# google/neural-light-transport

Hardware: AMD Instinct MI355X
Metric: rendered Mtexels/s at 1024^2 UV (full Model.call forward: U-Net + UV->camera warp); at N > 1: N collective-free replicas of this forward (weak scaling).  The data-parallel TRAIN step with the RCCL gradient all-reduce (BASELINE config 4) is `train_step`: value = Mtexels/s over all ranks, speedup_vs_o (higher is better)
Workload: dtype f32 via 3xbf16 split, 9 exact products, fp32 accumulate (the LDS-tiled encoder convs: fp32 operands as three bf16 terms on v_mfma_f32_16x16x32_bf16, every term product exact in fp32); f32 storage everywhere, every other launch native f32; 1 GPU; BASELINE config 3: dragon_specular relight+view-synth, depth0 16/depth 256, 4 frames/GPU, 1024^2 UV, k=4 obs maps, 512^2 camera warp; frames_per_gpu=4, uv=1024, k=4, cam=512, conv_algo=auto, plan=fused ends, launch=eager, two HIP streams, distinct_batches_rotated=3, launch_tape_replays=0, parallelism=dp1 (frames sharded, no forward collective), world=1, dist_world_size=1, device=cuda:0

## Files before the change

neural-light-transport_amd/_capi.py:

```python
import ctypes
import threading
import os

import torch

_HERE = os.path.dirname(os.path.abspath(__file__))
LIB_PATH = os.environ.get('NLT_HIP_LIB') or os.path.join(_HERE, 'libnlt_hip.so')

CONV1X1, CONV_K2S2, CONV_K2S1, DECONV_K2S2, DECONV_K2S1 = range(5)
CONV_K3S1, CONV_K3S2, DECONV_K3S1, DECONV_K3S2 = range(5, 9)
ALGO_AUTO, ALGO_DIRECT, ALGO_MFMA = range(3)

_c_int, _c_long, _c_float, _vp = ctypes.c_int, ctypes.c_long, ctypes.c_float, ctypes.c_void_p
_c_double = ctypes.c_double
MAP_F64, MAP_F32, MAP_F16 = range(3)

SIGNATURES = {
    'nlt_version': (ctypes.c_char_p, []),
    'nlt_status_string': (ctypes.c_char_p, [_c_int]),
    'nlt_packed_weight_floats': (_c_long, [_c_int] * 4),
    'nlt_pack_conv_weights': (_c_int, [_c_int, _vp, _c_int, _c_int, _c_int, _vp, _vp]),
    'nlt_conv_forward': (_c_int, [_c_int, _c_int, _c_int, _vp, _c_int, _c_int, _vp, _c_int, _c_int,
                                  _c_int, _c_int, _c_int, _vp, _vp, _vp, _c_int, _vp, _c_int,
                                  _c_int, _c_float, _vp, _c_int, _c_int, _vp]),
# ... 828 lines not shown


NORM_LAYER, NORM_BATCH = 0, 1


def norm_forward(kind, x, gamma, beta, mean, var, eps):
    c = x.shape[-1]
    y = torch.empty_like(x)
    _call('nlt_norm_forward', kind, _ptr(_dense(x, 'x')), x.numel() // c, c, _ptr(gamma), _ptr(beta), _ptr(mean), _ptr(var),
          float(eps), _ptr(y))
    return y


def norm_backward(kind, g, x, gamma, mean, var, eps, dgamma, dbeta):
    _same_shape(g, x, 'norm_backward')
    c = x.shape[-1]
    texels = x.numel() // c
    ws = _workspace('norm', x.device, _size('nlt_norm_workspace_floats', texels, c, what='the kernel takes c <= 1024'))
    dx = torch.empty_like(x)
    _call('nlt_norm_backward', kind, _ptr(_dense(g, 'g')), _ptr(_dense(x, 'x')), texels, c, _ptr(gamma), _ptr(mean), _ptr(var),
          float(eps), _ptr(dx), _ptr(dgamma), _ptr(dbeta), _ptr(ws))
    return dx


def pool2x2_forward(x, kind):
    n, h, w, c = x.shape
    y = torch.empty((n, h // 2, w // 2, c), device=x.device, dtype=torch.float32)
    _call('nlt_pool2x2_forward', _ptr(_dense(x, 'x')), n, h, w, c, kind, _ptr(y))
    return y


def pool2x2_backward(g, x, kind):
    n, h, w, c = x.shape
    if tuple(g.shape) != (n, h // 2, w // 2, c):
        raise NLTError("pool2x2_backward: gradient %s for input %s" % (tuple(g.shape), tuple(x.shape)))
    dx = torch.empty_like(x)
    _call('nlt_pool2x2_backward', _ptr(_dense(g, 'g')), _ptr(_dense(x, 'x')), n, h, w, c, kind, _ptr(dx))
    return dx


def clip_by_norm_slots(grad, slots, clipnorm):
    _call('nlt_clip_by_norm_slots', _ptr(grad), _tptr(slots, torch.int64, 'slots'), slots.shape[0], float(clipnorm))


def adam_amsgrad_step(param, grad, m, v, vhat, lr_t, beta1, beta2, eps):
    _call('nlt_adam_amsgrad_step', _ptr(param), _ptr(grad), _ptr(m), _ptr(v), _ptr(vhat), param.numel(), float(lr_t), float(beta1),
          float(beta2), float(eps))


def _splitk_workspace(mode, n, h, w, cout, ksplit, device, always=False):
    if abs(ksplit) <= 1 and not always:
        return None
    need = _size('nlt_conv_splitk_workspace_floats', mode, n, h, w, cout, ksplit)
    return _workspace((_stream(), getattr(_tls, 'scope', 0)), device, need, zero=True)


def conv_forward_splitk(mode, ksplit, src0, c0, ld0, src1, c1, ld1, n, h, w, w_packed, bias, cout, out, ldo,
                        act=True, alpha=0.3, tile_hint=0, mask_src=None, ldm=0, accumulate=False):
    ws = _splitk_workspace(mode, n, h, w, cout, ksplit, src0.device, always=True)
    _call('nlt_conv_forward_splitk', mode, tile_hint, ksplit, _ptr(ws), _ptr(src0), ld0, c0, _ptr(src1), ld1, c1, n, h, w,
          _ptr(w_packed), _ptr(bias), cout, _ptr(out), ldo, 1 if act else 0, float(alpha), _ptr(mask_src), ldm,
          1 if accumulate else 0)


def conv_forward_map(mode, ksplit, src0, c0, ld0, src1, c1, ld1, n, h, w, w_packed, bias, cout, out, ldo, bias_map,
                     act=True, alpha=0.3, tile_hint=0, w_keras=None):
    ws = _splitk_workspace(mode, n, h, w, cout, ksplit, src0.device)
    _call('nlt_conv_forward_map', mode, tile_hint, ksplit, _ptr(ws), _ptr(src0), ld0, c0, _ptr(src1), ld1, c1, n, h, w,
          _ptr(w_packed), _ptr(bias), cout, _ptr(out), ldo, 1 if act else 0, float(alpha), _ptr(_dense(bias_map, 'bias_map')),
          bias_map.shape[0])


def conv_backward_data(adj_mode, dpre, cpre, ldp, n, h, w, w_packed, zero_bias, cout, out, ldo, mask_src=None, ldm=0,
                       mask_alpha=0.3, accumulate=False, tile_hint=0, ksplit=1, split=None, w_keras=None):
    ws = _splitk_workspace(adj_mode, n, h, w, cout, ksplit, dpre.device)
    sc, sy, sd, sa, sp = split if split is not None else (0, None, None, 0.0, False)
    _call('nlt_conv_backward_data', adj_mode, tile_hint, ksplit, _ptr(ws), _ptr(dpre), ldp, cpre, n, h, w, _ptr(w_packed),
          _ptr(zero_bias), cout, _ptr(out), ldo, _ptr(mask_src), ldm, float(mask_alpha), 1 if accumulate else 0, sc, _ptr(sy),
          _ptr(sd), float(sa), 1 if sp else 0)


REPACK_MFMA, REPACK_TILE, REPACK_WINO, REPACK_TILE3S2 = 0, 1, 2, 3
REPACK_FIELDS = [('src', 'u8'), ('dst', 'u8'), ('total', 'i8'), ('first_block', 'i8'), ('kind', 'i4'), ('mode', 'i4'),
                 ('c0', 'i4'), ('c1', 'i4'), ('cout', 'i4'), ('tn', 'i4'), ('lo', 'i4'), ('full', 'i4')]


def repack_table(entries, device):
    import numpy as np
    tab = np.zeros(len(entries), dtype=np.dtype(REPACK_FIELDS))
    blocks = 0
    for i, e in enumerate(entries):
        nbytes = e['dst'].numel() * e['dst'].element_size()
        if nbytes % 16 or e['dst'].data_ptr() % 16:
            raise NLTError("repack_table: a packed buffer must be 16-byte aligned and a multiple of 4 floats long")
        tab[i] = (e['src'].data_ptr(), e['dst'].data_ptr(), nbytes // 4, blocks, e['kind'], e['mode'], e['c0'], e['c1'],
                  e['cout'], e['tn'], e['lo'], e['full'])
        blocks += (nbytes // 4 + 255) // 256
    return torch.from_numpy(tab.view(np.uint8)).to(device), len(entries), blocks


def repack_weights(table, n_desc, total_blocks):
    _call('nlt_repack_weights', _tptr(table, torch.uint8, 'repack table'), n_desc, total_blocks)


def conv_tile_supported(mode, cin, cout, tn):
    return lib().nlt_conv_tile_packed_floats(mode, cin, cout, tn) > 0

# ... 393 lines not shown
```

neural-light-transport_amd/csrc/conv_mfma.hip:

```cpp
#include "nlt_common.h"
#include "pack_common.h"

namespace {

typedef __attribute__((address_space(1))) unsigned gu32;

__host__ __device__ inline int chunks16(int c) { return (c + 15) >> 4; }

template <int MODE>
__device__ __forceinline__ int keras_widx(int t, int c, int ncol, int cin, int cout) {
  if (MODE == NLT_CONV1X1 || MODE == NLT_CONV_K2S2 || MODE == NLT_CONV_K2S1) return (t * cin + c) * cout + ncol;
  if (MODE == NLT_DECONV_K2S1) return (t * cout + ncol) * cin + c;
  return ncol * cin + c;
}

template <int MODE>
__global__ void pack_weights_kernel(const float* __restrict__ wk, int c0, int c1, int cout, int N,
                                    int ntiles, long total, float* __restrict__ wp) {
  const long idx = (long)blockIdx.x * blockDim.x + threadIdx.x;
  if (idx >= total) return;
  wp[idx] = nlt_mfma_fragment<MODE>(wk, idx, c0, c1, cout, N, ntiles, cout, 0);
}

template <int MODE>
// ... 106 lines not shown
        for (int rt = 0; rt < RT; ++rt)
#pragma unroll
          for (int ct = 0; ct < CT; ++ct)
            acc[rt][ct] = __builtin_amdgcn_mfma_f32_16x16x4f32(a_cur[ct][s4], b_cur[rt][s4], acc[rt][ct], 0, 0, 0);
#pragma unroll
      for (int ct = 0; ct < CT; ++ct) a_cur[ct] = a_nxt[ct];
#pragma unroll
      for (int rt = 0; rt < RT; ++rt) b_cur[rt] = b_nxt[rt];
    }

  } else {
    f32x4 af[PF][CT], bf[PF][RT];
    int t_n = kbeg / cps, r_n = kbeg - t_n * cps;
    int kload = kbeg;
    if (kbeg < kend) set_tap(t_n);
    auto issue = [&](f32x4 (&a)[CT], f32x4 (&b)[RT]) {
      const bool live = kload < kend;
      if (live && kload > kbeg) {
        if (++r_n == cps) { r_n = 0; set_tap(++t_n); }
      }
      load_frags(r_n, live ? kload : kend - 1, a, b);
      if (!live) {
#pragma unroll
        for (int rt = 0; rt < RT; ++rt) b[rt] = (f32x4){0.f, 0.f, 0.f, 0.f};
      }
      ++kload;
    };
    auto compute = [&](const f32x4 (&a)[CT], const f32x4 (&b)[RT]) {
#pragma unroll
      for (int s4 = 0; s4 < 4; ++s4)
#pragma unroll
        for (int rt = 0; rt < RT; ++rt)
#pragma unroll
          for (int ct = 0; ct < CT; ++ct)
            acc[rt][ct] = __builtin_amdgcn_mfma_f32_16x16x4f32(a[ct][s4], b[rt][s4], acc[rt][ct], 0, 0, 0);
    };
    if (kbeg < kend) {
#pragma unroll
      for (int j = 0; j < PF - 1; ++j) issue(af[j], bf[j]);
      for (int kc = kbeg; kc < kend; kc += PF) {
#pragma unroll
        for (int j = 0; j < PF; ++j) {
          issue(af[(j + PF - 1) % PF], bf[(j + PF - 1) % PF]);
          compute(af[j], bf[j]);
        }
      }
    }

  }
  if constexpr (SPLIT) {
    __shared__ f32x4 red[(NW - 1) * RT * CT * 64 + 1];
    const int kgroups = (ksplit + NW - 1) / NW;
    auto meet = [&]() {
      if (wv) {
#pragma unroll
        for (int rt = 0; rt < RT; ++rt)
#pragma unroll
          for (int ct = 0; ct < CT; ++ct) red[((wv - 1) * RT * CT + rt * CT + ct) * 64 + lane] = acc[rt][ct];
      }
      __syncthreads();
      if (!wv) {
#pragma unroll
        for (int j = 0; j < NW - 1; ++j)
#pragma unroll
          for (int rt = 0; rt < RT; ++rt)
#pragma unroll
            for (int ct = 0; ct < CT; ++ct) acc[rt][ct] += red[(j * RT * CT + rt * CT + ct) * 64 + lane];
      }
    };
    meet();
    if (kgroups > 1) {
      gu32* cnt = (gu32*)ws;
      float* slabs = ws + NLT_SPLITK_COUNTERS;
      const int npad = ntiles * 16;
      const size_t slab = (size_t)p.M * npad;
      if (!wv) {
#pragma unroll
        for (int ct = 0; ct < CT; ++ct) {
          const int ncol = (ng * CT + ct) * 16 + kk * 4;
#pragma unroll
          for (int rt = 0; rt < RT; ++rt)
            if (rv[rt]) *reinterpret_cast<f32x4*>(slabs + (size_t)kg * slab + (size_t)rm[rt] * npad + ncol) = acc[rt][ct];
        }
      }
      asm volatile("s_waitcnt vmcnt(0)" ::: "memory");
      __syncthreads();
      int* flag = reinterpret_cast<int*>(&red[(NW - 1) * RT * CT * 64]);
      if (threadIdx.x == 0) {
        __builtin_amdgcn_fence(__ATOMIC_RELEASE, "agent");
        asm volatile("s_waitcnt vmcnt(0)" ::: "memory");
        const unsigned t = __hip_atomic_fetch_add(cnt + tile, 1u, __ATOMIC_RELAXED, __HIP_MEMORY_SCOPE_AGENT);
        const int last = t == (unsigned)(kgroups - 1);
        if (last) __builtin_amdgcn_fence(__ATOMIC_ACQUIRE, "agent");
        *flag = last;
      }
      __syncthreads();
      if (!*flag) return;
#pragma unroll
      for (int rt = 0; rt < RT; ++rt)
#pragma unroll
        for (int ct = 0; ct < CT; ++ct) acc[rt][ct] = (f32x4){0.f, 0.f, 0.f, 0.f};
#pragma unroll(NW == 4 ? 4 : 1)
      for (int g = wv; g < kgroups; g += NW) {
#pragma unroll
        for (int ct = 0; ct < CT; ++ct) {
          const int ncol = (ng * CT + ct) * 16 + kk * 4;
#pragma unroll
          for (int rt = 0; rt < RT; ++rt)
            acc[rt][ct] += *reinterpret_cast<const f32x4*>(slabs + (size_t)g * slab + (size_t)rm[rt] * npad + ncol);
        }
      }
      meet();
      if (threadIdx.x == 0) __hip_atomic_store(cnt + tile, 0u, __ATOMIC_RELAXED, __HIP_MEMORY_SCOPE_AGENT);
    }
    if (wv) return;
  }

  if constexpr (!SPLIT) {
    if (ksplit > 1) {
      float* part = ws + NLT_SPLITK_COUNTERS;
      const int npad = ntiles * 16;
#pragma unroll
      for (int ct = 0; ct < CT; ++ct) {
        const int ncol = (ng * CT + ct) * 16 + kk * 4;
#pragma unroll
        for (int rt = 0; rt < RT; ++rt)
          if (rv[rt]) *reinterpret_cast<f32x4*>(part + ((size_t)ks * p.M + rm[rt]) * npad + ncol) = acc[rt][ct];
      }
      return;
    }
  }

#pragma unroll
  for (int ct = 0; ct < CT; ++ct) {
    const int ncol = (ng * CT + ct) * 16 + kk * 4;
    if (ncol >= p.N) continue;
    int oc = ncol, ab = 0;
    if (MODE == NLT_DECONV_K2S2) { ab = ncol / p.cout; oc = ncol - ab * p.cout; }
    const f32x4 bv = *reinterpret_cast<const f32x4*>(p.bias + oc);
#pragma unroll
    for (int rt = 0; rt < RT; ++rt) {
      if (!rv[rt]) continue;
      int otex = rm[rt];
      if (MODE == NLT_DECONV_K2S2) otex = (rf[rt] * p.oh + 2 * ry[rt] + (ab >> 1)) * p.ow + 2 * rx[rt] + (ab & 1);
      f32x4 v = acc[rt][ct] + bv;
      if (p.bmap) v += *reinterpret_cast<const f32x4*>(p.bmap + (size_t)(p.bmap_mod ? otex % p.bmap_mod : otex) * p.cout + oc);
      f32x4* o = reinterpret_cast<f32x4*>(p.out + (size_t)otex * p.ldo + oc);
      if (p.accumulate) v += *o;
      if (p.split_c && oc >= p.split_c) { split_store(p, otex, oc, v); continue; }
      if (p.mask_src) {
        const f32x4 mk = *reinterpret_cast<const f32x4*>(p.mask_src + (size_t)otex * p.ldm + oc);
#pragma unroll
        for (int j = 0; j < 4; ++j) v[j] *= (mk[j] > 0.f) ? 1.f : p.alpha;
      } else if (p.act) {
#pragma unroll
        for (int j = 0; j < 4; ++j) v[j] = v[j] > 0.f ? v[j] : p.alpha * v[j];
      }
      *o = v;
    }
  }
}

template <int MODE>
__device__ __forceinline__ void splitk_finish(const ConvP& p, int m, int ncol, f32x4 v) {
  int oc = ncol, ab = 0;
  if (MODE == NLT_DECONV_K2S2) { ab = ncol / p.cout; oc = ncol - ab * p.cout; }
  int otex = m;
  if (MODE == NLT_DECONV_K2S2) {
    const int x = m % p.gw, y = (m / p.gw) % p.gh, f = m / (p.gw * p.gh);
    otex = (f * p.oh + 2 * y + (ab >> 1)) * p.ow + 2 * x + (ab & 1);
  }
  v += *reinterpret_cast<const f32x4*>(p.bias + oc);
  if (p.bmap) v += *reinterpret_cast<const f32x4*>(p.bmap + (size_t)(p.bmap_mod ? otex % p.bmap_mod : otex) * p.cout + oc);
  f32x4* o = reinterpret_cast<f32x4*>(p.out + (size_t)otex * p.ldo + oc);
  if (p.accumulate) v += *o;
  if (p.split_c && oc >= p.split_c) { split_store(p, otex, oc, v); return; }
  if (p.mask_src) {
    const f32x4 mk = *reinterpret_cast<const f32x4*>(p.mask_src + (size_t)otex * p.ldm + oc);
#pragma unroll
    for (int j = 0; j < 4; ++j) v[j] *= (mk[j] > 0.f) ? 1.f : p.alpha;
  } else if (p.act) {
#pragma unroll
    for (int j = 0; j < 4; ++j) v[j] = v[j] > 0.f ? v[j] : p.alpha * v[j];
  }
  *o = v;
}

template <int MODE>
__global__ __launch_bounds__(256) void splitk_epilogue_kernel(ConvP p, int ntiles, int ksplit, const float* __restrict__ ws0) {
  const float* __restrict__ ws = ws0 + NLT_SPLITK_COUNTERS;
  const int quads = p.N >> 2;
  const long idx = (long)blockIdx.x * blockDim.x + threadIdx.x;
  if (idx >= (long)p.M * quads) return;
  const int m = idx / quads;
  const int ncol = (idx - (long)m * quads) * 4;
// ... 26 lines not shown
  }
  for (; ks < ksplit; ks += 8) s0 += *reinterpret_cast<const f32x4*>(src + (size_t)ks * slice);
  part[ksl][il] = (s0 + s1) + (s2 + s3);
  __syncthreads();
  if (ksl || !live) return;
  f32x4 v = part[0][il];
#pragma unroll
  for (int j = 1; j < 8; ++j) v += part[j][il];
  splitk_finish<MODE>(p, m, ncol, v);
}

int taps_of(int mode) { return (mode == NLT_CONV1X1 || mode == NLT_DECONV_K2S2) ? 1 : 4; }

template <int MODE, int RT, int CT>
int launch_tile(const ConvP& p, int ksplit, float* ws, hipStream_t s) {
  const int ntiles = (p.N + 15) >> 4;
  const int ngroups = ntiles / CT;
  const int mtiles = (p.M + 16 * RT - 1) / (16 * RT);
  const int total = live_taps<MODE>(p) * (chunks16(p.c0) + chunks16(p.c1));
  const bool two_launches = ksplit < 0;
  if (two_launches) ksplit = -ksplit;
  if (ksplit > total) ksplit = total;
  if (ksplit < 1 || !ws) ksplit = 1;
  const long tiles = (long)mtiles * ngroups;
  if (two_launches && ksplit > 1) {
    const unsigned blocks = (unsigned)((tiles * ksplit + 3) / 4);
    if ((total + ksplit - 1) / ksplit >= 24)
      hipLaunchKernelGGL((conv_mfma_kernel<MODE, RT, CT, 3, 0>), dim3(blocks), dim3(256), 0, s, p, mtiles, ngroups, ntiles, ksplit, ws);
    else
      hipLaunchKernelGGL((conv_mfma_kernel<MODE, RT, CT, 2, 0>), dim3(blocks), dim3(256), 0, s, p, mtiles, ngroups, ntiles, ksplit, ws);
    const long items = (long)p.M * (p.N >> 2);
    if (ksplit > 8)
      hipLaunchKernelGGL(splitk_epilogue_wide_kernel<MODE>, dim3((unsigned)((items + 31) / 32)), dim3(256), 0, s, p, ntiles, ksplit, ws);
    else
      hipLaunchKernelGGL(splitk_epilogue_kernel<MODE>, dim3((unsigned)((items + 255) / 256)), dim3(256), 0, s, p, ntiles, ksplit, ws);
    NLT_CHECK_LAUNCH();
    return NLT_OK;
  }
  if (ksplit > 4 && tiles > NLT_SPLITK_COUNTERS) ksplit = 4;
  const int per_wave = (total + ksplit - 1) / ksplit;
  if (ksplit > 1) {
    if constexpr (RT * CT <= 4) {
      if (ksplit >= 16) {
        const unsigned blocks = (unsigned)(tiles * ((ksplit + 15) >> 4));
        if (per_wave >= 24 && RT * CT <= 2)
          hipLaunchKernelGGL((conv_mfma_kernel<MODE, RT, CT, (RT * CT <= 2 ? 3 : 2), 16>), dim3(blocks), dim3(1024), 0, s, p, mtiles, ngroups, ntiles, ksplit, ws);
        else
          hipLaunchKernelGGL((conv_mfma_kernel<MODE, RT, CT, 2, 16>), dim3(blocks), dim3(1024), 0, s, p, mtiles, ngroups, ntiles, ksplit, ws);
        NLT_CHECK_LAUNCH();
        return NLT_OK;
      }
    }
    const unsigned blocks = (unsigned)(tiles * ((ksplit + 3) >> 2));
    if (per_wave >= 24)
      hipLaunchKernelGGL((conv_mfma_kernel<MODE, RT, CT, 3, 4>), dim3(blocks), dim3(256), 0, s, p, mtiles, ngroups, ntiles, ksplit, ws);
    else
      hipLaunchKernelGGL((conv_mfma_kernel<MODE, RT, CT, 2, 4>), dim3(blocks), dim3(256), 0, s, p, mtiles, ngroups, ntiles, ksplit, ws);
  } else {
    const unsigned blocks = (unsigned)((tiles + 3) / 4);
    if (per_wave >= 24)
      hipLaunchKernelGGL((conv_mfma_kernel<MODE, RT, CT, 3, 0>), dim3(blocks), dim3(256), 0, s, p, mtiles, ngroups, ntiles, 1, ws);
    else
      hipLaunchKernelGGL((conv_mfma_kernel<MODE, RT, CT, 2, 0>), dim3(blocks), dim3(256), 0, s, p, mtiles, ngroups, ntiles, 1, ws);
  }
  NLT_CHECK_LAUNCH();
  return NLT_OK;
}

template <int MODE>
int launch_mode(const ConvP& p, int tile_hint, int ksplit, float* ws, hipStream_t s) {
  const int ntiles = (p.N + 15) >> 4;
  int RT = 0, CT = 0;
  if (tile_hint > 0) { RT = tile_hint >> 4; CT = tile_hint & 15; }
  else {
    static const int cand[9][2] = {{4, 4}, {2, 4}, {4, 2}, {2, 2}, {1, 4}, {4, 1}, {1, 2}, {2, 1}, {1, 1}};
    RT = 1; CT = 1;
    for (int i = 0; i < 9; ++i) {
      const int r = cand[i][0], c = cand[i][1];
      if (ntiles % c) continue;
      const long waves = (long)((p.M + 16 * r - 1) / (16 * r)) * (ntiles / c);
      if (waves >= 2048) { RT = r; CT = c; break; }
    }
  }
  if (CT <= 0 || ntiles % CT) return NLT_ERR_UNSUPPORTED;
#define NLT_TILE(R, C) if (RT == R && CT == C) return launch_tile<MODE, R, C>(p, ksplit, ws, s);
  NLT_TILE(4, 4) NLT_TILE(2, 4) NLT_TILE(4, 2) NLT_TILE(2, 2) NLT_TILE(1, 4)
  NLT_TILE(4, 1) NLT_TILE(1, 2) NLT_TILE(2, 1) NLT_TILE(1, 1)
#undef NLT_TILE
  return NLT_ERR_UNSUPPORTED;
}

}

bool nlt_conv_mfma_supported(int mode, const ConvP& p) {
  (void)mode;
  if ((p.c0 & 3) || (p.c1 & 3) || (p.cout & 3) || (p.ld0 & 3) || (p.ldo & 3)) return false;
  if (p.c1 && (p.ld1 & 3)) return false;
  if (p.mask_src && (p.ldm & 3)) return false;
  if (!nlt_aligned16(p.src0) || !nlt_aligned16(p.out) || !nlt_aligned16(p.bias) || !nlt_aligned16(p.wgt)) return false;
  if (p.c1 && !nlt_aligned16(p.src1)) return false;
  if (p.mask_src && !nlt_aligned16(p.mask_src)) return false;
  return true;
}

int nlt_conv_mfma_launch(int mode, const ConvP& p, int tile_hint, hipStream_t s, int ksplit, float* ws) {
  if (!nlt_conv_mfma_supported(mode, p)) return NLT_ERR_UNSUPPORTED;
  switch (mode) {
    case NLT_CONV1X1: return launch_mode<NLT_CONV1X1>(p, tile_hint, ksplit, ws, s);
// ... 36 lines not shown
```

neural-light-transport_amd/engine.py:

```python
import os

import torch

from . import _capi as C
from .engine_infer import OverrideMixin


class OpTimer:

    def __init__(self):
        self.pending, self.records = [], {}
        self.flops = {}
        self.moved = {}

    def launch(self, label, nbytes, fn, *args, **kw):
        e0, e1 = torch.cuda.Event(enable_timing=True), torch.cuda.Event(enable_timing=True)
        e0.record()
        fn(*args, **kw)
        e1.record()
        self.pending.append((label, nbytes, e0, e1))

    def collect(self):
        torch.cuda.synchronize()
        for label, nbytes, e0, e1 in self.pending:
            r = self.records.setdefault(label, [0, 0.0, nbytes])
            r[0] += 1
            r[1] += e0.elapsed_time(e1)
        self.pending = []
        return self.records


def _act_kw(act):
    return {'act': act is not None, 'alpha': act.alpha if act is not None else 0.0}


def _gemm(mode, n, h, w, cin, cout):
    ncols = cout * (4 if mode == C.DECONV_K2S2 else 1)
    taps = 4 if mode in (C.CONV_K2S2, C.CONV_K2S1, C.DECONV_K2S1) else 1
    rows = n * h * w // (4 if mode == C.CONV_K2S2 else 1)
    return rows, ncols, 2 * rows * taps * cin * ncols


CHOICE_DICTS = {'tile': ('tile_hints',), 'direct': ('algo_hints',), 'lds': ('lds_hints',), 'splitk': ('tile_hints', 'splitk_hints'),
                'wino': ('wino_hints',), 'c32': ('c32_hints',)}
HINT_DICTS = tuple(dict.fromkeys(a for attrs in CHOICE_DICTS.values() for a in attrs))
EXCLUSIVE = ('lds', 'wino', 'c32')


def hint_word(hint):
    return hint & 255, bool(hint & 256), bool(hint & 512)


FOLD_S2 = 1024
FOLD_HINT = FOLD_S2 + 512 + 32


class RenderPlan(OverrideMixin):
    def __init__(self, net_query, net_obs, use_obs=True):
        self.timer = None
        self.q, self.o, self.use_obs = net_query, net_obs, use_obs
        self.tile_hints = {}
        self.algo_hints = {}
        self.lds_hints = {}
        self.splitk_hints = {}
        self.wino_hints = {}
        self.c32_hints = {}
        self._trial = None
        self._ran = set()
        self.autotune = os.environ.get('NLT_AUTOTUNE', '1') != '0'
        self.fuse_ends = os.environ.get('NLT_FUSED', '1') != '0'
        self._front_blob = None
        self.fuse_override = os.environ.get('NLT_FUSED_OVERRIDE', '1') != '0'
        self._ovr = None
        self.front_l2 = os.environ.get('NLT_FRONT_L2', '1') != '0'
        self.fuse_dec = os.environ.get('NLT_FUSED_DEC', '1') != '0'
        self.front_v4 = os.environ.get('NLT_FRONT4', '1') != '0'
        self.fuse_train = os.environ.get('NLT_FUSED_TRAIN', '1') != '0'
        self.front4_train = os.environ.get('NLT_FRONT4_TRAIN', '1') != '0'
        self.two_streams = os.environ.get('NLT_STREAMS', '2') != '1'
        self._side = None
        self._bside = None
        self.wgrad_tiled = os.environ.get('NLT_WGRAD', 'tiled') != 'atomic'
        self.wgrad_narrow = os.environ.get('NLT_WGRAD_NARROW', '1') != '0'
        self.bwd_streams = int(os.environ.get('NLT_BWD_STREAMS', '1'))
        self.use_tape = os.environ.get('NLT_TAPE', '1') != '0'
        self.fold_split = os.environ.get('NLT_FOLD_SPLIT', '1') != '0'
        self.tile_dgrad = os.environ.get('NLT_TILE_DGRAD', '1') != '0'
        self._tuning = False
        self.tune_backward = os.environ.get('NLT_TUNE_BWD', '1') != '0'
        self.precision = os.environ.get('NLT_PRECISION', 'fp32')
        self._pred_out = None
        self._pred_slot = 'back_infer'
        self.prune_packs = os.environ.get('NLT_PRUNE_PACKS', '1') != '0'
        self.grad_hook = None
        self.grad_mid_level = 0
        self.generation = 0
        self.tape_replays = 0
        self.use_wino = os.environ.get('NLT_WINO', '1') != '0'
        self.use_c32 = os.environ.get('NLT_C32', '1') != '0'
        self.fold_s2 = os.environ.get('NLT_FOLD_S2', '1') != '0'
        self.alias_obs = os.environ.get('NLT_ALIAS_OBS', '1') != '0'
        is_c = net_query.is_contracting
        self.n_down = sum(is_c) - 1
        self.n_up = len(is_c) - sum(is_c) - 1
        assert self.n_down == self.n_up
        self._bufs = {}

    def __del__(self):
        try:
            C.drop_workspace_scope(id(self))
        except Exception:
            pass

    def _buffers(self, n, k, h, w, device):
        key = (n, k, h, w, str(device), self.precision)
        b = self._bufs.get(key)
        if b is not None:
            return b
        bf = self.precision == 'bf16'
        E = lambda *s, lo=False: torch.empty(s, device=device, dtype=torch.bfloat16 if (bf and lo) else torch.float32)
# ... 10 lines not shown
                b['qtmp'].append(E(n, hh, ww, cl[l], lo=l >= 3))
                b['otmp'].append(E(n, k, hh, ww, cl[l], lo=l >= 3))
            b['fm'].append(E(n, hh, ww, mult * cl[l], lo=l >= 3))
            b['obs'].append(E(n, k, hh, ww, cl[l], lo=l >= 3))
        for j in range(self.n_up):
            nl = q.layers[D + 1 + j].convs()[0][0].n_ch_out
            hh, ww = hh * 2, ww * 2
            b['dtmp'].append(E(n, hh, ww, nl, lo=j <= D - 3))
            b['dec'].append(E(n, hh, ww, nl, lo=j < D - 3))
        b['pred'] = E(n, h, w, 3)
        b['skip3'] = None
        self._bufs = {key: b}
        return b

    def _level_channels(self):
        q = self.q
        return [q.layers[0].n_ch_out] + [q.layers[l].convs()[0][0].n_ch_out for l in range(1, self.n_down + 1)]

    def _launch(self, label, nbytes, fn, *args, flops=0, moved=None, **kw):
        t = self.timer
        if t is not None:
            t.flops[label] = flops
            if moved is not None:
                t.moved[label] = moved
        if t is not None and (getattr(t, 'only', None) is None or label in t.only):
            t.launch(label, nbytes, fn, *args, **kw)
        else:
            fn(*args, **kw)

    def _trying(self, kind):
        return self._trial is not None and self._trial[0] == kind

    def _hint(self, kind, label):
        if self._trial is not None:
            return self._trial[1] if self._trial[0] == kind else 0
        return getattr(self, CHOICE_DICTS[kind][0]).get(label, 0)

    def ran(self, kind):
        return {label for label, k in self._ran if k == kind}

    def set_choice(self, label, kind, hint):
        own = [getattr(self, a) for a in CHOICE_DICTS[kind]]
        rivals = [getattr(self, CHOICE_DICTS[k][0]) for k in EXCLUSIVE] if kind in EXCLUSIVE else []
        if any(label in d for d in own + rivals):
            return
        values = (C.ALGO_DIRECT,) if kind == 'direct' else hint if kind == 'splitk' else (hint,)
        for d, v in zip(own, values):
            d[label] = v

    def clear_choices(self):
        for a in HINT_DICTS:
            setattr(self, a, {})

    def _tile_splitk(self, label, rows, ncols, star, ok=True):
        kind, hint = self._trial or (None, 0)
        if kind is None:
            tile_hint, ks = self.tile_hints.get(label, self.tile_hints.get('*', 0) if star else 0), self.splitk_hints.get(label, 1)
        else:
            tile_hint, ks = (hint if kind == 'tile' else hint[0] if kind == 'splitk' else 0), 1
        if tile_hint and ((ncols + 15) // 16) % (tile_hint & 15):
            tile_hint = 0
        if kind == 'splitk' and ok:
            rt, ct = (tile_hint >> 4, tile_hint & 15) if tile_hint else (1, 1)
            waves = -(-rows // (16 * rt)) * (-(-ncols // 16) // ct)
            npad = -(-ncols // 16) * 16
            ks = hint[1] if (waves < 4096 and rows * npad * abs(hint[1]) <= (1 << 24)) else 1
        return tile_hint, ks

    def _conv(self, label, layer, act, src0, c0, ld0, src1, c1, ld1, n, h, w, out, ldo, algo=C.ALGO_AUTO, bmap=None):
        layer.build(c0 + c1, src0.device)
        assert layer.cin == c0 + c1, (layer.cin, c0, c1)
        small = (c0 + c1) * layer.n_ch_out <= 1024
        if self._hint('direct', label) == C.ALGO_DIRECT or (self._trying('direct') and small):
            algo = C.ALGO_DIRECT
            self._ran.add((label, 'direct'))
        ok = c0 % 4 == 0 and c1 % 4 == 0 and layer.n_ch_out % 4 == 0 and algo != C.ALGO_DIRECT
        oh, ow = layer.out_hw(h, w)
        nbytes = 4 * (n * h * w * (c0 + c1) + n * oh * ow * layer.n_ch_out)
        rows, ncols, flops = _gemm(layer.mode, n, h, w, c0 + c1, layer.n_ch_out)
        if c1 == 0 and ok and algo == C.ALGO_AUTO and self._wino(label, layer, act, src0, c0, ld0, n, 1, h, w, out, ldo):
            return
        tile_hint, ks = self._tile_splitk(label, rows, ncols, True, ok)
        srcs = (src0, c0, ld0, src1, c1, ld1, n, h, w)
        dst = (layer.bias.detach(), layer.n_ch_out, out, ldo)
        kw = dict(_act_kw(act), flops=flops)
        if bmap is not None:
            if not ok:
                raise C.NLTError("a bias-map conv needs channel counts that are multiples of 4 (%s)" % label)
            if abs(ks) > 1:
                self._ran.add((label, 'splitk'))
            self._launch(label, nbytes, C.conv_forward_map, layer.mode, ks or 1, *srcs, layer.packed(c0, c1), *dst, bmap,
                         tile_hint=tile_hint, w_keras=layer.kernel.detach(), **kw)
        elif abs(ks) > 1 and ok:
            self._ran.add((label, 'splitk'))
            self._launch(label, nbytes, C.conv_forward_splitk, layer.mode, ks, *srcs, layer.packed(c0, c1), *dst,
                         tile_hint=tile_hint, **kw)
        else:
            self._launch(label, nbytes, C.conv_forward, layer.mode, *srcs, layer.kernel.detach(),
                         layer.packed(c0, c1) if ok else None, *dst, algo=algo if ok else C.ALGO_DIRECT,
                         tile_hint=tile_hint if ok else 0, **kw)

    def _mean(self, label, obs, obs_weights, frames, kobs, hw, c, mean_out, ldm):
        self._launch(label.replace('.s1', '.mean'), 4 * frames * hw * c * (kobs + 1), C.obs_mean_forward,
                     obs, obs_weights, frames, kobs, hw, c, mean_out, ldm)

    def _enc_launch(self, fn, packed, extra, kind, unfold, label, layer, act, src, cin, ld, frames, kobs, h, w, out, ldo,
                    mean_out, ldm, **kw):
        oh, ow = layer.out_hw(h, w)
        nf, c = frames * kobs, layer.n_ch_out
        fold_mean = mean_out is not None and not unfold
        nbytes = 4 * (nf * h * w * cin + nf * oh * ow * c)
        if fold_mean:
            nbytes += 4 * frames * oh * ow * c * (kobs + 1)
        self._ran.add((label, kind))
        self._launch(label, nbytes, fn, layer.mode, src, ld, cin, nf if unfold else frames, 1 if unfold else kobs, h, w, packed,
                     layer.bias.detach(), c, *extra, out, ldo, mean_out if fold_mean else None, ldm, **_act_kw(act), **kw,
                     flops=2 * nf * oh * ow * 4 * cin * c)
        if mean_out is not None and unfold:
            self._mean(label, out, None, frames, kobs, oh * ow, c, mean_out, ldm)

    def _wino(self, label, layer, act, src, cin, ld, frames, kobs, h, w, out, ldo, mean_out=None, ldm=0, obs_weights=None):
        tn, unfold, _ = hint_word(self._hint('wino', label))
        if not (tn and self.use_wino and obs_weights is None and layer.mode in (C.CONV_K2S1, C.DECONV_K2S1) and layer.cin == cin
                and cin % 8 == 0 and layer.n_ch_out % tn == 0 and ld % 4 == 0 and ldo % 4 == 0):
            return False
        if layer.mode == C.DECONV_K2S1 and (kobs > 1 or mean_out is not None):
            return False
        if kobs == 1 and mean_out is None:
            if unfold and self._trial is not None:
                return False
            unfold = False
        self._enc_launch(C.conv_wino_forward, layer.packed_wino(tn), (tn,), 'wino', unfold, label, layer, act, src, cin, ld,
                         frames, kobs, h, w, out, ldo, mean_out, ldm)
        return True

# ... 52 lines not shown
                if mean_out is None and kobs == 1:
                    mean_out, ldm = out, ldo
                self._conv_fold(label, layer, act, src, cin, ld, frames, kobs, h, w, mean_out, ldm, fold)
                return True
            ok = ok and not trial
        if ok and resident and (self.precision not in ('f32x3', 'f32x3_9') or C.conv_tile3r_plan(layer.mode, cin, tn) is None):
            ok = not trial
            resident = False
        if ok and unfold and kobs == 1:
            ok = not trial
            unfold = False
        if ok and self.precision in ('f32x3', 'f32x3_9'):
            self._enc_launch(C.conv_tile3r_forward if resident else C.conv_tile3_forward, layer.packed_tile3(tn), (tn,),
                             'lds', unfold, *conv, nprod=9 if self.precision == 'f32x3_9' else 6)
        elif ok:
            self._enc_launch(C.conv_tile_forward, layer.packed_tile(tn), (tn,), 'lds', unfold, *conv)
        else:
            self._conv(label, layer, act, src, cin, ld, None, 0, 0, frames * kobs, h, w, out, ldo, algo)
            if mean_out is not None:
                oh, ow = layer.out_hw(h, w)
                self._mean(label, out, obs_weights, frames, kobs, oh * ow, layer.n_ch_out, mean_out, ldm)

    def _dec_block_plain(self, b, j, lab, da, dact_a, db, dact_b, srcs, n, hh, ww, algo, s2_label=None, bmap=None):
        nl = da.n_ch_out
        self._conv(s2_label or lab + '.s2', da, dact_a, *srcs, n, hh, ww, b['dtmp'][j], nl, algo, bmap=bmap)
        self._conv(lab + '.s1', db, dact_b, b['dtmp'][j], nl, nl, None, 0, 0, n, 2 * hh, 2 * ww, b['dec'][j], db.n_ch_out, algo)
        return b['dec'][j], db.n_ch_out

    def _autotune(self, run, backward=False):
        saved_timer = self.timer
        self._tuning = True
        results = {}
        trials = [('tile', 16 * r + c) for r in (1, 2, 4) for c in (1, 2, 4)]
        if not self.fuse_ends and not backward:
            trials.append(('direct', 0))
        if not backward:
            trials += [('lds', 32), ('lds', 64), ('lds', 256 + 32), ('lds', 256 + 64)]
            if self.precision in ('f32x3', 'f32x3_9'):
                trials += [('lds', 512 + 32), ('lds', 512 + 64)]
                if self.fold_s2 and self._fold_trial():
                    trials.append(('lds', FOLD_HINT))
        elif self.tile_dgrad:
            trials += [('lds', 32), ('lds', 64)]
        if self.use_c32 and not backward:
            trials += [('c32', 1), ('c32', 2)]
        if self.use_wino:
            trials += [('wino', 32), ('wino', 64)] + ([('wino', 256 + 32), ('wino', 256 + 64)] if not backward else [])
        mode = os.environ.get('NLT_SPLITK', 'all')
        if mode == 'all' or (mode == 'fwd' and not backward):
            forms = os.environ.get('NLT_SPLITK_FORMS', 'both')
            cand = ((4, 8, 16, 32, 64, 128) if forms != 'two' else ()) + ((-16, -32, -64, -128) if forms == 'both' else ()) + \
                   ((-4, -8, -16, -32, -64, -128) if forms == 'two' else ())
            trials += [('splitk', (16 * r + c, ks)) for (r, c) in ((1, 1), (1, 2), (2, 2), (1, 4)) for ks in cand]
        try:
            for kind, hint in trials:
                self._trial, self._ran = (kind, hint), set()
                self.timer = None
                run()
                self.timer = OpTimer()
                run(); run()
                rec = self.timer.collect()
                for label, r in rec.items():
                    t = r[1] / r[0]
                    if label.endswith('.o.s1') and label.replace('.s1', '.mean') in rec:
                        m = rec[label.replace('.s1', '.mean')]
                        t += m[1] / m[0]
                    if kind == 'tile' or (label, kind) in self._ran:
                        results.setdefault(label, []).append((t, kind, hint))
        finally:
            self._trial, self.timer, self._tuning = None, saved_timer, False
        for label, res in results.items():
            t_fold = [t for t, kind, hint in res if kind == 'lds' and hint == FOLD_HINT]
            label2 = self._fold_partner(label)
            if t_fold and not backward and label2 in results:
                rest = [r for r in res if not (r[1] == 'lds' and r[2] == FOLD_HINT)]
                if rest and min(t_fold) < min(rest)[0] + min(results[label2])[0]:
                    self.set_choice(label, 'lds', FOLD_HINT)
        for label, res in results.items():
            if '.s1' not in label and '.s2' not in label and label != 'L0.q':
                continue
            _, kind, hint = min(r for r in res if not (r[1] == 'lds' and r[2] == FOLD_HINT))
            if backward and 'dgrad' not in label:
                continue
            self.set_choice(label, kind, hint)
        self.tuned = {**getattr(self, 'tuned', {}), **results}
        self._drop_tapes()
        reg = getattr(self.q.layers[0], '_registry', None)
        if reg is not None and self.prune_packs:
            reg.begin_census()

    def _fold_trial(self):
        k = getattr(self.q.layers[0], 'kernel', None)
        return k is not None and k.is_cuda

    @staticmethod
    def _fold_partner(label):
        parts = label.split('.')
        if len(parts) != 3 or parts[1:] != ['o', 's1'] or not parts[0][1:].isdigit():
            return None
        return 'L%d.o.s2' % (int(parts[0][1:]) + 1)

    def _drop_tapes(self):
        for b in self._bufs.values():
            b.pop('tapes', None)

    def export_tuning(self):
        return {a: dict(getattr(self, a)) for a in HINT_DICTS}

# ... 427 lines not shown
            ev = events[cur[0]]
            if len(bs) > 3 and bs[3] is not None and cur[0] % 2:
                side = bs[3]
            cur[0] += 1
            C.record_event(ev, torch.cuda.current_stream())
            with torch.cuda.stream(side):
                C.wait_event(side, ev)
                self._wgrad_now(label, layer, src0, c0, ld0, src1, c1, ld1, n, h, w, dpre, ldp)
            return
        self._wgrad_now(label, layer, src0, c0, ld0, src1, c1, ld1, n, h, w, dpre, ldp)

    def _grad_range_done(self, i):
        bs = self._bside
        if bs is not None and bs[2] is not None and bs[3] is not None:
            side, events, cur, side2 = bs
            if cur[0] == len(events):
                events.append(C.new_event())
            C.record_event(events[cur[0]], side2)
            C.wait_event(side, events[cur[0]])
            cur[0] += 1
        C.tape_call(self._fire_grad_hook, bs[0] if (bs is not None and bs[2] is not None) else None, i)

    def _fire_grad_hook(self, side, i=0):
        hook = self.grad_hook
        if hook is None or self._tuning:
            return
        if side is not None:
            with torch.cuda.stream(side):
                hook(i)
        else:
            hook(i)

    def _wgrad_now(self, label, layer, src0, c0, ld0, src1, c1, ld1, n, h, w, dpre, ldp):
        oh, ow = layer.out_hw(h, w)
        nbytes = 4 * (n * h * w * (c0 + c1) + n * oh * ow * layer.n_ch_out)
        gw = w // 2 if layer.mode == C.CONV_K2S2 else w
        tiled = (self.wgrad_tiled and c0 % 4 == 0 and c1 % 4 == 0 and layer.n_ch_out % 4 == 0 and ld0 % 4 == 0
                 and (c1 == 0 or ld1 % 4 == 0) and ldp % 4 == 0 and gw >= 4)
        fn = C.conv_backward_weights_tiled if tiled else C.conv_backward_weights
        ncols = layer.n_ch_out * (4 if layer.mode == C.DECONV_K2S2 else 1)
        kdim = (c0 + c1) * (1 if layer.mode in (C.DECONV_K2S2, C.CONV1X1) else 4)
        if self.wgrad_narrow and ncols <= 32 and kdim <= 128 and layer.mode != C.CONV1X1 and gw >= 4:
            fn = C.conv_backward_weights_narrow
        self._launch(label, nbytes, fn, layer.mode, src0, c0, ld0, src1, c1, ld1, n, h, w,
                     dpre, ldp, layer.n_ch_out, layer.dkernel, layer.dbias)

    def _dgrad(self, label, layer, lo, hi, dpre, ldp, n, oh, ow, out, ldo, mask_src=None, ldm=0, mask_alpha=0.3,
               accumulate=False, zero_bias=None, split=None):
        packed, ks = layer.packed_adjoint(lo, hi)
        adj = layer.ADJOINT[layer.mode]
        out_px = n * oh * ow * (4 if adj == C.DECONV_K2S2 else 1) // (4 if adj == C.CONV_K2S2 else 1)
        nbytes = 4 * (n * oh * ow * layer.n_ch_out + out_px * (hi - lo))
        rows, ncols, flops = _gemm(adj, n, oh, ow, layer.n_ch_out, hi - lo)
        tile_hint, nks = self._tile_splitk(label, rows, ncols, False)
        wtn = hint_word(self._hint('wino', label))[0]
        if (wtn and self.use_wino and split is None and adj in (C.CONV_K2S1, C.DECONV_K2S1) and layer.n_ch_out % 8 == 0
                and (hi - lo) % wtn == 0 and ldp % 4 == 0 and ldo % 4 == 0 and layer.kernel.is_contiguous()):
            self._ran.add((label, 'wino'))
            self._launch(label, nbytes, C.conv_wino_backward_data, adj, dpre, layer.n_ch_out, ldp, n, oh, ow,
                         layer.packed_adjoint_wino(lo, hi, wtn), hi - lo, wtn, out, ldo, mask_src=mask_src, ldm=ldm,
                         mask_alpha=mask_alpha, accumulate=accumulate, flops=flops)
            return
        tn = hint_word(self._hint('lds', label))[0]
        tile_ok = tn and ldp % 4 == 0 and ldo % 4 == 0 and layer.kernel.is_contiguous()
        if tile_ok and adj == C.DECONV_K2S2:
            tile_ok = layer.n_ch_out % 32 == 0 and (hi - lo) % 16 == 0 and (4 * (hi - lo)) % tn == 0
        elif tile_ok:
            tile_ok = (split is None and adj in (C.CONV_K2S1, C.CONV_K2S2, C.DECONV_K2S1) and layer.n_ch_out % 16 == 0
                       and (hi - lo) % tn == 0)
        if tile_ok:
            self._ran.add((label, 'lds'))
            self._launch(label, nbytes, C.conv_tile_backward_data, adj, dpre, layer.n_ch_out, ldp, n, oh, ow,
                         layer.packed_adjoint_tile(lo, hi, tn), hi - lo, tn, out, ldo, mask_src=mask_src, ldm=ldm, mask_alpha=mask_alpha,
                         accumulate=accumulate, split=split, w_keras=ks, flops=flops)
            return
        if abs(nks) > 1:
            self._ran.add((label, 'splitk'))
        self._launch(label, nbytes, C.conv_backward_data, adj, dpre, layer.n_ch_out, ldp, n, oh, ow, packed, zero_bias, hi - lo,
                     out, ldo, mask_src=mask_src, ldm=ldm, mask_alpha=mask_alpha, accumulate=accumulate, tile_hint=tile_hint,
                     ksplit=nks, split=split, w_keras=ks, flops=flops)

    def backward(self, dpred, base, cvis, lvis, nn_rgb, nn_base, obs_weights=None, generation=None):
        C.set_workspace_scope(id(self))
        if generation is not None and generation != self.generation:
            raise RuntimeError("backward() of a forward pass whose activations have been overwritten by a later forward "
                               "(pass %d, the plan now holds pass %d): run each backward before the next forward"
                               % (generation, self.generation))
        n, h, w, _ = base.shape
        k = nn_rgb.shape[1]
        b = self._buffers(n, k, h, w, base.device)
        g = self._grad_buffers(b)
        reg = self._begin_pass(bump=False, refresh=False)
        run = lambda: self._backward_streams(dpred, base, cvis, lvis, nn_rgb, nn_base, obs_weights, b, g, n, h, w, k)
        if self.tune_backward and not self._tuning and self._tune_once(b, 'tuned_bwd', dpred.is_cuda, run, backward=True):
            bucket = getattr(self.q.layers[0].dkernel, '_base', None)
            if bucket is not None:
                bucket.zero_()
        tkey = None
        if (self._tape_ok(reg, dpred.is_cuda) and obs_weights is None
                and all(t.is_contiguous() for t in (dpred, base, cvis, lvis, nn_rgb, nn_base))):
            tkey = ('bwd', dpred.data_ptr(), base.data_ptr(), cvis.data_ptr(), lvis.data_ptr(), nn_rgb.data_ptr(),
                    nn_base.data_ptr(), bool(b.get('train_fused')), self.bwd_streams, C._stream(), C.deterministic())
        self._run_taped(b, reg, tkey, run, valid=lambda b, ent, reg: C.tape_valid(ent, reg.version), finish=lambda b: None)

    def _backward_streams(self, dpred, base, cvis, lvis, nn_rgb, nn_base, obs_weights, b, g, n, h, w, k):
        concurrent = self.bwd_streams and dpred.is_cuda and self.timer is None
        if concurrent:
# ... 137 lines not shown
```

Before: 3755 Mtexels/s.

## Distribute split-K reduction across waves and autotune tall split-K tiles

The in-block split-K reduction now spreads fragments round-robin across all waves instead of funnelling everything through wave 0. Each wave reduces, writes slabs and runs the epilogue for its own fragments. The autotuner gains extra split-K trials with taller tiles (2x4, 4x2, 4x4), run only for layers whose estimated weight-stream volume is large. Pipeline depth is reduced to 2 for the largest tiles to limit register pressure. The changes aim to cut the serial reduction and epilogue bottleneck on one wave and to reuse weights better on weight-bound layers, at the cost of more tuning time and added complexity.

```diff
diff --git a/neural-light-transport_amd/_capi.py b/neural-light-transport_amd/_capi.py
--- a/neural-light-transport_amd/_capi.py
+++ b/neural-light-transport_amd/_capi.py
@@ -904,7 +904,10 @@
     if abs(ksplit) <= 1 and not always:
         return None
     need = _size('nlt_conv_splitk_workspace_floats', mode, n, h, w, cout, ksplit)
-    return _workspace((_stream(), getattr(_tls, 'scope', 0)), device, need, zero=True)
+    ws = _workspace((_stream(), getattr(_tls, 'scope', 0)), device, need, zero=True)
+    if ws.numel() < need:
+        raise NLTError("split-K scratch of %d floats, the launch needs %d" % (ws.numel(), need))
+    return ws
 
 
 def conv_forward_splitk(mode, ksplit, src0, c0, ld0, src1, c1, ld1, n, h, w, w_packed, bias, cout, out, ldo,
diff --git a/neural-light-transport_amd/csrc/conv_mfma.hip b/neural-light-transport_amd/csrc/conv_mfma.hip
--- a/neural-light-transport_amd/csrc/conv_mfma.hip
+++ b/neural-light-transport_amd/csrc/conv_mfma.hip
@@ -182,20 +182,20 @@
     __shared__ f32x4 red[(NW - 1) * RT * CT * 64 + 1];
     const int kgroups = (ksplit + NW - 1) / NW;
     auto meet = [&]() {
-      if (wv) {
-#pragma unroll
-        for (int rt = 0; rt < RT; ++rt)
-#pragma unroll
-          for (int ct = 0; ct < CT; ++ct) red[((wv - 1) * RT * CT + rt * CT + ct) * 64 + lane] = acc[rt][ct];
+#pragma unroll
+      for (int f = 0; f < RT * CT; ++f) {
+        const int o = f % NW;
+        if (wv != o) red[(f * (NW - 1) + (wv < o ? wv : wv - 1)) * 64 + lane] = acc[f / CT][f % CT];
       }
       __syncthreads();
-      if (!wv) {
-#pragma unroll
-        for (int j = 0; j < NW - 1; ++j)
-#pragma unroll
-          for (int rt = 0; rt < RT; ++rt)
-#pragma unroll
-            for (int ct = 0; ct < CT; ++ct) acc[rt][ct] += red[(j * RT * CT + rt * CT + ct) * 64 + lane];
+#pragma unroll
+      for (int f = 0; f < RT * CT; ++f) {
+        const int o = f % NW;
+        if (wv != o) continue;
+        f32x4 v = o ? red[f * (NW - 1) * 64 + lane] : acc[f / CT][f % CT];
+#pragma unroll
+        for (int j = 1; j < NW; ++j) v += j == o ? acc[f / CT][f % CT] : red[(f * (NW - 1) + (j < o ? j : j - 1)) * 64 + lane];
+        acc[f / CT][f % CT] = v;
       }
     };
     meet();
@@ -204,14 +204,13 @@
       float* slabs = ws + NLT_SPLITK_COUNTERS;
       const int npad = ntiles * 16;
       const size_t slab = (size_t)p.M * npad;
-      if (!wv) {
-#pragma unroll
-        for (int ct = 0; ct < CT; ++ct) {
-          const int ncol = (ng * CT + ct) * 16 + kk * 4;
-#pragma unroll
-          for (int rt = 0; rt < RT; ++rt)
-            if (rv[rt]) *reinterpret_cast<f32x4*>(slabs + (size_t)kg * slab + (size_t)rm[rt] * npad + ncol) = acc[rt][ct];
-        }
+#pragma unroll
+      for (int ct = 0; ct < CT; ++ct) {
+        const int ncol = (ng * CT + ct) * 16 + kk * 4;
+#pragma unroll
+        for (int rt = 0; rt < RT; ++rt)
+          if ((rt * CT + ct) % NW == wv && rv[rt])
+            *reinterpret_cast<f32x4*>(slabs + (size_t)kg * slab + (size_t)rm[rt] * npad + ncol) = acc[rt][ct];
       }
       asm volatile("s_waitcnt vmcnt(0)" ::: "memory");
       __syncthreads();
@@ -243,8 +242,8 @@
       meet();
       if (threadIdx.x == 0) __hip_atomic_store(cnt + tile, 0u, __ATOMIC_RELAXED, __HIP_MEMORY_SCOPE_AGENT);
     }
-    if (wv) return;
-  }
+  }
+  auto mine = [&](int f) { return !SPLIT || f % (SPLIT ? NW : 1) == wv; };
 
   if constexpr (!SPLIT) {
     if (ksplit > 1) {
@@ -270,7 +269,7 @@
     const f32x4 bv = *reinterpret_cast<const f32x4*>(p.bias + oc);
 #pragma unroll
     for (int rt = 0; rt < RT; ++rt) {
-      if (!rv[rt]) continue;
+      if (!rv[rt] || !mine(rt * CT + ct)) continue;
       int otex = rm[rt];
       if (MODE == NLT_DECONV_K2S2) otex = (rf[rt] * p.oh + 2 * ry[rt] + (ab >> 1)) * p.ow + 2 * rx[rt] + (ab & 1);
       f32x4 v = acc[rt][ct] + bv;
@@ -403,8 +402,8 @@
       }
     }
     const unsigned blocks = (unsigned)(tiles * ((ksplit + 3) >> 2));
-    if (per_wave >= 24)
-      hipLaunchKernelGGL((conv_mfma_kernel<MODE, RT, CT, 3, 4>), dim3(blocks), dim3(256), 0, s, p, mtiles, ngroups, ntiles, ksplit, ws);
+    if (per_wave >= 24 && RT * CT < 16)
+      hipLaunchKernelGGL((conv_mfma_kernel<MODE, RT, CT, (RT * CT < 16 ? 3 : 2), 4>), dim3(blocks), dim3(256), 0, s, p, mtiles, ngroups, ntiles, ksplit, ws);
     else
       hipLaunchKernelGGL((conv_mfma_kernel<MODE, RT, CT, 2, 4>), dim3(blocks), dim3(256), 0, s, p, mtiles, ngroups, ntiles, ksplit, ws);
   } else {
diff --git a/neural-light-transport_amd/engine.py b/neural-light-transport_amd/engine.py
--- a/neural-light-transport_amd/engine.py
+++ b/neural-light-transport_amd/engine.py
@@ -45,6 +45,21 @@
                 'wino': ('wino_hints',), 'c32': ('c32_hints',)}
 HINT_DICTS = tuple(dict.fromkeys(a for attrs in CHOICE_DICTS.values() for a in attrs))
 EXCLUSIVE = ('lds', 'wino', 'c32')
+
+
+TALL_TILES = ((2, 4), (4, 2), (4, 4))
+TALL_SLICES = (4, 8, 16, 32)
+TALL_MIN_STREAM = 16 << 20
+
+
+def weight_stream_bytes(rows, flops):
+    return -(-rows // 16) * (2 * flops // max(rows, 1))
+
+
+def tall_splitk_trials(wstream):
+    if not any(b >= TALL_MIN_STREAM for b in wstream.values()):
+        return []
+    return [('splitk', (16 * r + c, ks)) for (r, c) in TALL_TILES for ks in TALL_SLICES]
 
 
 def hint_word(hint):
@@ -66,6 +81,7 @@
         self.wino_hints = {}
         self.c32_hints = {}
         self._trial = None
+        self._wstream = {}
         self._ran = set()
         self.autotune = os.environ.get('NLT_AUTOTUNE', '1') != '0'
         self.fuse_ends = os.environ.get('NLT_FUSED', '1') != '0'
@@ -182,8 +198,10 @@
         for a in HINT_DICTS:
             setattr(self, a, {})
 
-    def _tile_splitk(self, label, rows, ncols, star, ok=True):
+    def _tile_splitk(self, label, rows, ncols, star, ok=True, flops=0):
         kind, hint = self._trial or (None, 0)
+        if self._tuning and flops:
+            self._wstream[label] = weight_stream_bytes(rows, flops)
         if kind is None:
             tile_hint, ks = self.tile_hints.get(label, self.tile_hints.get('*', 0) if star else 0), self.splitk_hints.get(label, 1)
         else:
@@ -195,6 +213,8 @@
             waves = -(-rows // (16 * rt)) * (-(-ncols // 16) // ct)
             npad = -(-ncols // 16) * 16
             ks = hint[1] if (waves < 4096 and rows * npad * abs(hint[1]) <= (1 << 24)) else 1
+            if (rt, ct) in TALL_TILES and self._wstream.get(label, 0) < TALL_MIN_STREAM:
+                ks = 1
         return tile_hint, ks
 
     def _conv(self, label, layer, act, src0, c0, ld0, src1, c1, ld1, n, h, w, out, ldo, algo=C.ALGO_AUTO, bmap=None):
@@ -210,7 +230,7 @@
         rows, ncols, flops = _gemm(layer.mode, n, h, w, c0 + c1, layer.n_ch_out)
         if c1 == 0 and ok and algo == C.ALGO_AUTO and self._wino(label, layer, act, src0, c0, ld0, n, 1, h, w, out, ldo):
             return
-        tile_hint, ks = self._tile_splitk(label, rows, ncols, True, ok)
+        tile_hint, ks = self._tile_splitk(label, rows, ncols, True, ok, flops)
         srcs = (src0, c0, ld0, src1, c1, ld1, n, h, w)
         dst = (layer.bias.detach(), layer.n_ch_out, out, ldo)
         kw = dict(_act_kw(act), flops=flops)
@@ -369,8 +389,16 @@
             cand = ((4, 8, 16, 32, 64, 128) if forms != 'two' else ()) + ((-16, -32, -64, -128) if forms == 'both' else ()) + \
                    ((-4, -8, -16, -32, -64, -128) if forms == 'two' else ())
             trials += [('splitk', (16 * r + c, ks)) for (r, c) in ((1, 1), (1, 2), (2, 2), (1, 4)) for ks in cand]
+        tall = (mode == 'all' or (mode == 'fwd' and not backward)) and os.environ.get('NLT_SPLITK_FORMS', 'both') != 'two'
+        tall = tall and os.environ.get('NLT_SPLITK_TALL', '1') != '0'
+        self._wstream = {}
+
+        def staged():
+            yield from trials
+            if tall:
+                yield from tall_splitk_trials(self._wstream)
         try:
-            for kind, hint in trials:
+            for kind, hint in staged():
                 self._trial, self._ran = (kind, hint), set()
                 self.timer = None
                 run()
@@ -904,7 +932,7 @@
         out_px = n * oh * ow * (4 if adj == C.DECONV_K2S2 else 1) // (4 if adj == C.CONV_K2S2 else 1)
         nbytes = 4 * (n * oh * ow * layer.n_ch_out + out_px * (hi - lo))
         rows, ncols, flops = _gemm(adj, n, oh, ow, layer.n_ch_out, hi - lo)
-        tile_hint, nks = self._tile_splitk(label, rows, ncols, False)
+        tile_hint, nks = self._tile_splitk(label, rows, ncols, False, flops=flops)
         wtn = hint_word(self._hint('wino', label))[0]
         if (wtn and self.use_wino and split is None and adj in (C.CONV_K2S1, C.DECONV_K2S1) and layer.n_ch_out % 8 == 0
                 and (hi - lo) % wtn == 0 and ldp % 4 == 0 and ldo % 4 == 0 and layer.kernel.is_contiguous()):
```

Result: no change. 3750 Mtexels/s (median of 2 runs) (-0.1%).
